# vpc-ccg/freddie

Measured on AMD Instinct MI355X. Metric: reads segmented/sec (whole node), higher is better.
Workload: dtype u32

## Files before the change

freddie_amd/csrc/freddie_seg.hip:

```cpp
#include "seg_kernels.h"

using namespace fseg;

namespace {

struct DevBuf {
    void *p = nullptr;
    size_t cap = 0;
    template <typename T> T *as() const { return reinterpret_cast<T *>(p); }
};
struct Slab {
    void *p = nullptr;
    size_t cap = 0;
};
struct HostBuf {
    void *p = nullptr;
    size_t cap = 0;
    template <typename T> T *as() const { return reinterpret_cast<T *>(p); }
};
struct Carve {
    struct Item { DevBuf *b; size_t off, bytes; };
    std::vector<Item> items;
    size_t total = 0;
    size_t add(DevBuf &b, size_t bytes) {
// ... 20 lines not shown
    SEG_POST1 = 8u,
    SEG_POST2 = 16u,
    SEG_STATUS = 32u,
    SEG_ALL = 63u,
};

}

hipError_t fseg_sort_pairs(void *tmp, size_t *tmp_bytes, const unsigned long long *keys_in, unsigned long long *keys_out,
                           const int *vals_in, int *vals_out, size_t n, unsigned end_bit, hipStream_t stream);

struct fseg_ctx {
    int device = 0;
    hipStream_t stream = nullptr;
    std::string err;
    bool have_params = false, have_batch = false, ran = false, pending = false;
    bool fetched = false;
    fseg_params P{};
    std::vector<double> w_main, w_refine, h_table;
    int n_part = 0;
    i64 K = 0, R = 0, I = 0, NPOS = 0, LANES = 0;
    i64 max_part_pos = 0;
    int thr_part = -1;
    i64 max_part_lanes = 0;
    int n_tiles = 0;
    bool expanded = false;
    std::vector<i64> part_iv_off, part_rep_off;
    Slab slab_in, slab_pos, slab_arena;
    HostBuf h_stage;
    HostBuf h_res;
    size_t res_off[4] = {0, 0, 0, 0};
    std::vector<i64> res_pfo;
    DevBuf d_labels;
    DevBuf d_packed;
    int fetched_packed = -1;
    bool label_packed_ok = true;
    bool label_has2 = false;
    bool run_label_packed = false;
    bool labels_unpacked = false;
    DevBuf d_sort_tmp;
    DevBuf d_part_iv_off, d_part_rep_off, d_part_lane_off, d_iv_start, d_iv_end, d_pos_off, d_iv_part,
        d_rep_exon_off, d_rep_weight, d_ex_ts, d_ex_te, d_tile_desc, d_iv_tile0, d_blk_iv0, d_rb_part, d_rb_r0, d_rb_sum, d_rb_base, d_rb_max, d_rb_cmax,
        d_hc_part, d_hc_p0, d_hc_n, d_hc_glo, d_hc_ghi;
    DevBuf d_lane_ex, d_lane_start, d_lane_pmax, d_hc_llo, d_hc_lhi, d_key_a, d_key_b, d_val_a, d_val_b, d_rep_last;
    DevBuf d_lane_lx, d_lex, d_rb_esum, d_rb_ebase;
    i64 max_rep_exons = 0;
    DevBuf d_w_main, d_w_refine, d_h_table, d_thr_tab;
    DevBuf d_bits;
    DevBuf d_y_raw, d_y, d_v, d_scan_state, d_bsum, d_bsum_side, d_g, d_pk, d_pf, d_kp;
    int n_hist_chunks = 0;
    DevBuf d_voff, d_chunk_off, d_csum, d_mean, d_thr, d_label_off, d_part_has2;
    int n_rep_blocks = 0;
    DevBuf d_cand_off, d_cand_y, d_fixed0, d_added, d_fixed, d_chosen, d_final_off, d_final_y, d_final_pos, d_final_iv, d_col_thr,
        d_col_zero;
    DevBuf d_tile_defer;
    DevBuf d_blk_pre, d_tile_tot, d_seg_iv, d_seg_prev, d_rseg_c, d_cand_pn, d_cand_ll, d_cand_ln, d_cand_wide, d_prob_bs;
    DevBuf d_prob_iv, d_prob_start, d_prob_n, d_prob_pair_off, d_prob_tri_off, d_prob_flags, d_prob_chain,
        d_prob_cov_off, d_prob_lane_lo, d_prob_lane_n;
    DevBuf d_dp_items, d_solve_items, d_solve_desc, d_prob_desc, d_work_pc, d_cls_items, d_work_active, d_pair_thr, d_amb, d_out, d_cov;
    DevBuf d_wide_items;
    DevBuf d_wide_all;
    DevBuf d_dpx;
    i64 dpx_base[3] = {0, 0, 0}, dpx_stride[3] = {0, 0, 0}, dpx_n[3] = {0, 0, 0};
    int dpx_nm = 0, dpx_cnt[3] = {1, 1, 1};
    static constexpr i64 kWideOneMax = 256;
    int split_dp = 7;
    i64 prob_cap = 0, work_cap = 0, pair_cap = 0, tri_cap = 0, label_cap = 0, chunk_cap = 0, cov_cap = 0;
    DevBuf d_status, d_prep, d_tacc;
    DevBuf d_sync;
    unsigned sync_gen = 0;
    unsigned sync_ticks = 1000000u;
    unsigned sync_timeouts = 0;
    unsigned forked_runs = 0;
    bool run_events_only = false;
    bool dev_sync = true;
    Status *h_status = nullptr;
    PrepStatus *h_prep = nullptr;
    bool prep_checked = false;
    bool counted_in_flight = false, counted_live = false;
    bool side_probed = false;
    bool side_ok[3] = {false, false, false};
    unsigned probe_gen = 0;
    bool owns_device = false;
    int hsa_agent = -1;
    hsa_signal_t hsa_sig = {0};
    int hsa_cpu = 0;
    const void *hsa_dst_base = nullptr;
    bool profiling = false;
    bool profile_all = true;
    bool have_huge = false;
    int nm_giant = 0;
    DevBuf d_giant;
    bool dp_wide_counts = false;
    int nm_big = kNMax;
    bool small_batch = false;
    bool tiny_on = false;
    bool use_graph = true;
    bool run_plain = false;
    bool run_linear = false;
    bool use_sized = true;
    static constexpr i64 kProbSelfMax = 4 * kProbBlock;
    bool prob_self_scan = false;
    i64 scan_single_max = 512;
    bool force_scan_stall = false;
    hipGraph_t graph[2] = {nullptr, nullptr};
    hipGraphExec_t graph_exec[2] = {nullptr, nullptr};
    bool profile_plain = false;
// ... 619 lines not shown
                           c->d_pair_thr.as<int2>(), c->pair_cap, c->P.min_read_support_outside, c->d_chosen.as<unsigned char>(), 0); \
              \
        hipLaunchKernelGGL((k_dp<kDpSmall, 256, OUTT>), dim3(grid_for(c->prob_cap, 1, 8192)), dim3(256),                       \
                           dp_lds_for(kDpSmall, (int)sizeof(OUTT)), q_mid, st, 0, kDpSmall, c->d_dp_items.as<int>(), pr,       \
                           c->d_prob_desc.as<ProbDesc>(), c->prob_cap, c->d_cand_off.as<i64>(), c->d_cand_y.as<int>(), c->d_iv_part.as<int>(), \
                           c->d_part_lane_off.as<i64>(), c->d_out.as<unsigned>(), c->tri_cap, c->d_amb.as<unsigned>(),        \
                           c->d_pair_thr.as<int2>(), c->pair_cap, c->P.min_read_support_outside,                              \
                           c->d_chosen.as<unsigned char>(), kDpWave, grid_for(c->prob_cap, 1, 8192), (uint4 *)nullptr, (i64)0 FSEG_TARG)
        hipStream_t q_small = c->small_batch ? s : fork(0);
        hipStream_t q_mid = c->small_batch ? s : fork(1);
        if (c->dp_wide_counts) {
            const bool wide_wg = dp_lds_for(c->nm_big, 4) + 8 * 1024 <= kLdsPerWg;
            if (!c->small_batch) { FSEG_LAUNCH_DP_WAVES(unsigned); }
            if (wide_wg) { FSEG_LAUNCH_DP(kNMax, 512, unsigned, c->nm_big, c->small_batch ? -1 : 1, 256); }
            else { FSEG_LAUNCH_DP(kNMax, 256, unsigned, c->nm_big, c->small_batch ? -1 : 1, 256); }
        } else {
            if (!c->small_batch) { FSEG_LAUNCH_DP_WAVES(unsigned short); }
            FSEG_LAUNCH_DP(kNMax, 512, unsigned short, c->nm_big, c->small_batch ? -1 : 1, 512);
        }
#undef FSEG_LAUNCH_DP
#undef FSEG_LAUNCH_DP_WAVES
        if (!c->small_batch) { join(0); join(1); }
        if (c->have_huge)
            hipLaunchKernelGGL(k_dp_huge, dim3(dp_grid < 256 ? dp_grid : 256), dim3(512), kHugeDpLds, s, st, c->d_dp_items.as<int>(),
                               pr, c->d_prob_desc.as<ProbDesc>(), c->prob_cap, c->d_cand_y.as<int>(), c->d_out.as<unsigned>(),
                               c->tri_cap, c->d_amb.as<unsigned>(), c->d_pair_thr.as<int2>(), c->pair_cap,
                               c->P.min_read_support_outside, c->d_chosen.as<unsigned char>());
        if (c->have_huge && c->nm_giant > 0 && c->d_giant.p)
            hipLaunchKernelGGL(k_dp_giant, dim3(kGiantWgs), dim3(512), giant_dp_lds(c->nm_giant), s, st, c->d_dp_items.as<int>(),
                               pr, c->d_prob_desc.as<ProbDesc>(), c->prob_cap, c->d_cand_y.as<int>(), c->d_out.as<unsigned>(),
                               c->tri_cap, c->d_amb.as<unsigned>(), c->d_pair_thr.as<int2>(), c->pair_cap,
                               c->P.min_read_support_outside, c->d_chosen.as<unsigned char>(), c->nm_giant,
                               c->d_giant.as<unsigned char>(), (i64)giant_scratch_bytes(c->nm_giant));
    }
    end(ST_DP); begin(ST_REFINE);
    hipLaunchKernelGGL(k_segments, dim3(grid_for(K, 1, 8192)), dim3(iv_threads), 0, s, K, c->d_pos_off.as<i64>(),
                       c->d_cand_off.as<i64>(), c->d_cand_y.as<int>(), c->d_y_raw.as<int>(), c->d_blk_pre.as<int>(), c->d_tile_tot.as<int>(), c->d_iv_tile0.as<int>(),
                       c->d_chosen.as<unsigned char>(), flag_final_bits, c->d_rseg_c.as<int>(),
                       c->d_seg_prev.as<int>(), st);
    hipLaunchKernelGGL(k_refine, dim3(2048), dim3(64), 0, s, st, c->d_seg_iv.as<int>(), c->d_rseg_c.as<int>(),
                       c->d_seg_prev.as<int>(), c->d_cand_y.as<int>(), c->d_pos_off.as<i64>(), c->d_y_raw.as<int>(),
                       c->d_w_refine.as<double>(), c->P.radius_refine, c->P.sigma, c->d_g.as<double>(), c->d_pk.as<int>(),
                       c->d_pf.as<unsigned char>(), c->d_kp.as<unsigned char>(), flag_final_bits);
    end(ST_REFINE); begin(ST_FINAL);
    scan_counts(s, bsum, flag_final_bits, &st->n_final, c->d_final_off.as<i64>() + K);
    hipLaunchKernelGGL(k_scan_emit<kEmitPositions>, dim3(scan_grid), dim3(256), 0, s, flag_final_bits,
                       NPOS, bsum, scan_state + 2 * scan_nb, &st->n_final, c->d_final_off.as<i64>() + K, &st->err, (const double *)nullptr, (double *)nullptr, K, c->d_pos_off.as<i64>(),
                       c->d_iv_start.as<int>(), c->d_blk_iv0.as<int>(), c->d_final_y.as<int>(), c->d_final_pos.as<int>(),
                       c->d_final_off.as<i64>(), 0, c->d_final_iv.as<int>());
    hipLaunchKernelGGL(k_label_cols, dim3(grid_for(NPOS / 8 + 1, 256, 2048)), dim3(256), 0, s, K, c->d_final_off.as<i64>(),
                       c->d_final_y.as<int>(), c->d_final_iv.as<int>(), c->d_iv_part.as<int>(), c->d_h_table.as<double>(), c->P.h_len,
                       c->P.threshold_rate, c->d_thr_tab.as<int2>(), c->d_col_thr.as<int2>(), c->d_col_zero.as<unsigned char>(),
                       c->d_part_has2.as<int>(), n_part, c->d_part_iv_off.as<i64>(), c->d_part_rep_off.as<i64>(),
                       c->d_label_off.as<i64>(), st, c->label_cap);
    end(ST_FINAL);
    }
    if (do_post2) {
    begin(ST_LABEL);
    if (c->label_cap > 0) {
        c->run_label_packed = lab_packed; c->labels_unpacked = false;
        if (lab_packed) {
            const i64 n16 = sized ? (label_fill_bytes + 15) / 16 : labels_n16;
            if (n16 > 0)
                hipLaunchKernelGGL(k_clear, dim3(grid_for(n16 / 4 + 1, 256, 4096)), dim3(256), 0, s, (Status *)nullptr, c->d_packed.as<unsigned>(), n16);
        } else if (!ride_fill) {
            const i64 n16 = sized ? (label_fill_bytes + 15) / 16 : labels_n16;
            if (n16 > 0)
                hipLaunchKernelGGL(k_label_zero, dim3(grid_for(n16 / 8 + 1, 256, 4096)), dim3(256), 0, s, c->d_labels.as<uint4>(), n16);
        }
        hipLaunchKernelGGL(k_label_reads, dim3(grid_for((i64)c->n_rep_blocks * kLabelSplit, 1, 65536)), dim3(256), 0, s, c->n_rep_blocks,
                           c->d_rb_part.as<int>(), c->d_rb_r0.as<int>(), c->d_label_off.as<i64>(), c->label_cap, n_part,
                           c->d_part_iv_off.as<i64>(), c->d_part_rep_off.as<i64>(), c->d_final_off.as<i64>(),
                           c->d_final_pos.as<int>(), c->d_col_thr.as<int2>(), c->d_rep_exon_off.as<i64>(),
                           c->d_ex_ts.as<int>(), c->d_ex_te.as<int>(), c->d_col_zero.as<unsigned char>(),
                           c->d_part_has2.as<int>(), c->d_labels.as<unsigned char>(), lab_packed ? c->d_packed.as<unsigned>() : (unsigned *)nullptr);
    }
    end(ST_LABEL);
    }
    if (segs & SEG_STATUS) HIP_TRY(c, hipMemcpyAsync(c->h_status, st, sizeof(Status), hipMemcpyDeviceToHost, s));
    HIP_TRY(c, fj_err);
    HIP_TRY(c, hipGetLastError());
    return FSEG_OK;
}

hipError_t wait_stream(fseg_ctx *c) {
    const auto t0 = std::chrono::steady_clock::now();
    for (;;) {
        hipError_t e = hipStreamQuery(c->stream);
        if (e != hipErrorNotReady) { (void)hipGetLastError(); return e; }
        if (std::chrono::steady_clock::now() - t0 > std::chrono::milliseconds(2)) break;
    }
    (void)hipGetLastError();
    return hipStreamSynchronize(c->stream);
}

int check_prep(fseg_ctx *c) {
    if (c->prep_checked) return FSEG_OK;
    c->prep_checked = true;
    const PrepStatus &ps = *c->h_prep;
    if (!ps.err) return FSEG_OK;
    int q = 0;
    for (int i = 1; i < 4; ++i) if (((ps.err >> i) & 1u) && (!((ps.err >> q) & 1u) || ps.bad_rep[i] < ps.bad_rep[q])) q = i;
    if (!((ps.err >> q) & 1u)) for (q = 0; q < 4 && !((ps.err >> q) & 1u); ++q) {}
    const long long r = (long long)ps.bad_rep[q];
    c->have_batch = false;
    switch (1u << q) {
        case kPrepExonEnds: return fail(c, FSEG_ERR_INPUT, "rep %lld: exon with start >= end (py/freddie_segment.py:160)", r);
        case kPrepExonOrder: return fail(c, FSEG_ERR_INPUT, "rep %lld: exons out of order (py/freddie_segment.py:158)", r);
        case kPrepExonInterval: return fail(c, FSEG_ERR_INPUT, "rep %lld: an exon does not lie inside one tint interval (py/freddie_segment.py:668)", r);
        default: return fail(c, FSEG_ERR_INPUT, "rep %lld has no exons", r);
    }
}

int run_input_errors(fseg_ctx *c, const Status &s) {
    if (s.err & kErrExonInterval) return fail(c, FSEG_ERR_INPUT, "an exon does not lie inside one tint interval (py/freddie_segment.py:668)");
    if (s.err & kErrBreakAssert) return fail(c, FSEG_ERR_INPUT, "break_large_problems: candidate window out of range or no positive signal (py/freddie_segment.py:640-643)");
    if (s.err & kErrWideMissed) return fail(c, FSEG_ERR_HIP, "internal: a problem keeps more reads than were counted for it (kErrWideMissed)");
    if (s.err & kErrProblemTooLarge) return fail(c, FSEG_ERR_UNSUPPORTED, "a DP problem has more than %d candidates (max_problem_size beyond 1000 is not supported)", kNGiant);
    return FSEG_OK;
}

int prepare_giant(fseg_ctx *c, int max_n) {
    if (max_n <= kNHuge || max_n > kNGiant) { if (max_n <= kNHuge) c->nm_giant = 0; return FSEG_OK; }
    int want = (max_n + 7) & ~7;
    if (want > kNGiant) want = kNGiant;
    if (want > c->nm_giant || c->nm_giant == 0) { c->nm_giant = want; drop_graph(c); }
    TRY(ensure(c, c->d_giant, (size_t)kGiantWgs * giant_scratch_bytes(c->nm_giant)));
    const hipError_t e = hipFuncSetAttribute(reinterpret_cast<const void *>(k_score_giant), hipFuncAttributeMaxDynamicSharedMemorySize, (int)giant_score_lds(kNGiant));
// ... 603 lines not shown
            TRY(ensure(c, c->d_sort_tmp, tmp_bytes));
            HIP_TRY(c, fseg_sort_pairs(c->d_sort_tmp.p, &tmp_bytes, c->d_key_a.as<u64>(), c->d_key_b.as<u64>(), c->d_val_a.as<int>(),
                                       c->d_val_b.as<int>(), (size_t)R, end_bit, s));
        }
        if (sort_here) {
            hipLaunchKernelGGL(k_lanes, dim3(grid_for(np, 1, 65536)), dim3(256), 0, s, np, c->d_part_rep_off.as<i64>(), c->d_part_lane_off.as<i64>(),
                               c->d_key_b.as<u64>(), c->d_val_b.as<int>(), c->d_rep_weight.as<int>(), c->d_rep_last.as<int>(),
                               c->d_rep_exon_off.as<i64>(), c->d_lane_ex.as<longlong2>(), c->d_lane_start.as<int>(), c->d_lane_pmax.as<int>(),
                               1, c->d_key_a.as<u64>(), c->d_ex_ts.as<int>(), c->d_ex_te.as<int>(), c->d_lane_lx.as<int2>(), c->d_lex.as<int2>());
        } else {
            const int rbg = grid_for(n_rep_blocks, 1, 65536);
            hipLaunchKernelGGL(k_lane_blocks, dim3(rbg), dim3(256), 0, s, (int)n_rep_blocks, c->d_rb_part.as<int>(), c->d_rb_r0.as<int>(),
                               c->d_part_rep_off.as<i64>(), c->d_val_b.as<int>(), c->d_rep_weight.as<int>(), c->d_rep_last.as<int>(),
                               c->d_rb_sum.as<i64>(), c->d_rb_max.as<int>(), c->d_rep_exon_off.as<i64>(), c->d_rb_esum.as<i64>());
            hipLaunchKernelGGL(k_lane_block_scan, dim3(grid_for(np, 4, 4096)), dim3(256), 0, s, np, (int)n_rep_blocks, c->d_rb_part.as<int>(),
                               c->d_part_lane_off.as<i64>(), c->d_rb_sum.as<i64>(), c->d_rb_max.as<int>(), c->d_rb_base.as<i64>(),
                               c->d_rb_cmax.as<int>(), c->d_part_rep_off.as<i64>(), c->d_rep_exon_off.as<i64>(), c->d_rb_esum.as<i64>(),
                               c->d_rb_ebase.as<i64>());
            hipLaunchKernelGGL(k_lane_emit, dim3(rbg), dim3(256), 0, s, (int)n_rep_blocks, c->d_rb_part.as<int>(), c->d_rb_r0.as<int>(),
                               c->d_part_rep_off.as<i64>(), c->d_key_b.as<u64>(), c->d_val_b.as<int>(), c->d_rep_weight.as<int>(),
                               c->d_rep_last.as<int>(), c->d_rep_exon_off.as<i64>(), c->d_rb_base.as<i64>(), c->d_rb_cmax.as<int>(),
                               c->d_lane_ex.as<longlong2>(), c->d_lane_start.as<int>(), c->d_lane_pmax.as<int>(), c->d_rb_ebase.as<i64>(),
                               c->d_ex_ts.as<int>(), c->d_ex_te.as<int>(), c->d_lane_lx.as<int2>(), c->d_lex.as<int2>());
        }
    }
    hipLaunchKernelGGL(k_hist_ranges, dim3(grid_for(n_chunks, 256, 4096)), dim3(256), 0, s, (int)n_chunks, c->d_hc_part.as<int>(),
                       c->d_hc_glo.as<int>(), c->d_hc_ghi.as<int>(), c->d_part_lane_off.as<i64>(), c->d_lane_start.as<int>(),
                       c->d_lane_pmax.as<int>(), c->d_hc_llo.as<i64>(), c->d_hc_lhi.as<i64>());
    HIP_TRY(c, hipMemcpyAsync(c->h_prep, c->d_prep.p, sizeof(PrepStatus), hipMemcpyDeviceToHost, s));
    HIP_TRY(c, hipGetLastError());
    {
        const size_t np8 = (size_t)NPOS + 64;
        auto atleast = [](i64 &cap, i64 v) { if (cap < v) cap = v; };
        atleast(c->chunk_cap, NPOS / 8192 + np + 8);
        Carve cv;
        cv.add(c->d_y_raw, np8 * 4); cv.add(c->d_y, np8 * 8); cv.add(c->d_bits, 3 * flag_words(np8) * 4);
        cv.add(c->d_v, np8 * 8);
        cv.add(c->d_scan_state, ((size_t)nb * 3 + 1) * 8);
        cv.add(c->d_bsum, ((size_t)nb + 2) * 4);
        cv.add(c->d_bsum_side, ((size_t)nb + 2) * 4);
        cv.add(c->d_g, np8 * 8); cv.add(c->d_pk, np8 * 4); cv.add(c->d_pf, np8); cv.add(c->d_kp, np8);
        cv.add(c->d_part_has2, ((size_t)np + 1) * 4);
        cv.add(c->d_tile_tot, ((size_t)n_tiles + 1) * 4);
        cv.add(c->d_blk_pre, ((size_t)n_tiles + 1) * (kSmoothTile / kSumBlock) * 4);
        cv.add(c->d_tile_defer, ((size_t)n_tiles + 1) * 4);
        cv.add(c->d_voff, ((size_t)np + 2) * 8); cv.add(c->d_chunk_off, ((size_t)np + 2) * 8);
        cv.add(c->d_mean, ((size_t)np + 1) * 8); cv.add(c->d_thr, ((size_t)np + 1) * 8);
        cv.add(c->d_label_off, ((size_t)np + 2) * 8);
        cv.add(c->d_csum, (size_t)c->chunk_cap * 16);
        cv.add(c->d_cand_off, ((size_t)K + 2) * 8); cv.add(c->d_final_off, ((size_t)K + 2) * 8);
        cv.add(c->d_cand_y, np8 * 4); cv.add(c->d_fixed0, np8); cv.add(c->d_added, np8);
        cv.add(c->d_fixed, np8); cv.add(c->d_chosen, np8);
        cv.add(c->d_final_y, np8 * 4); cv.add(c->d_final_pos, np8 * 4); cv.add(c->d_final_iv, np8 * 4); cv.add(c->d_col_thr, np8 * 8); cv.add(c->d_col_zero, np8);
        cv.add(c->d_seg_iv, np8 * 4); cv.add(c->d_seg_prev, np8 * 4); cv.add(c->d_rseg_c, np8 * 4);
        cv.add(c->d_cand_pn, np8 * 4); cv.add(c->d_cand_ll, np8 * 4); cv.add(c->d_cand_ln, np8 * 4); cv.add(c->d_cand_wide, np8);
        cv.add(c->d_prob_bs, ((size_t)NPOS / kProbBlock + 2) * kProbCols * 8);
        TRY(reserve(c, c->slab_pos, cv.total));
        cv.bind(c->slab_pos);
        atleast(c->prob_cap, 1024); atleast(c->work_cap, 1024); atleast(c->pair_cap, 1 << 16); atleast(c->tri_cap, 1 << 18);
        atleast(c->label_cap, 1 << 16); atleast(c->cov_cap, 1 << 18);
        TRY(alloc_arenas(c));
    }
    drop_graph(c);
    c->have_batch = true;
    if (c->trace)
        fprintf(stderr, "[fseg] upload: plan %.3f ms, tables %.3f ms, copy-in %.3f ms (%.1f MB), enqueue %.3f ms; %lld positions, %lld reps, %lld exons\n",
                t_plan, t_tables, t_copy, up_bytes / 1e6, tk.ms(), (long long)NPOS, (long long)R, (long long)I);
    return FSEG_OK;
}

static int run_impl(fseg_ctx *c);
int fseg_run(fseg_ctx *c) {
    const int rc = run_impl(c);
    if (rc != FSEG_OK && c && !c->pending) set_in_flight(c, false);
    return rc;
}
static int run_impl(fseg_ctx *c) {
    if (!c) return FSEG_ERR_ARG;
    if (!c->have_params || !c->have_batch) return fail(c, FSEG_ERR_ARG, "fseg_run: set parameters and upload a batch first");
    HIP_TRY(c, hipSetDevice(c->device));
    if (c->pending) TRY(finish_run(c));
    c->fetched = false;
    c->run_events_only = false;
    set_in_flight(c, true);
    claim_device(c);
    if (c->owns_device) ++c->forked_runs;
    if (c->use_fork && !c->side[0] && c->owns_device) {
        hipStream_t made[fseg_ctx::kSide] = {};
        hipError_t e = hipSuccess;
        for (int i = 0; e == hipSuccess && i < fseg_ctx::kSide; ++i) e = hipStreamCreateWithFlags(&made[i], hipStreamNonBlocking);
        if (e != hipSuccess) {
            for (hipStream_t m : made) if (m) (void)hipStreamDestroy(m);
            return fail(c, FSEG_ERR_HIP, "hipStreamCreateWithFlags: %s", hipGetErrorString(e));
        }
        for (int i = 0; i < fseg_ctx::kSide; ++i) c->side[i] = made[i];
    }
    if (c->owns_device && c->dev_sync && !c->side_probed) TRY(probe_side_queues(c));
    if (!c->ran && c->use_sized) return run_sized(c);
    if (c->label_cap > 0) {
        void *before[2] = {c->d_labels.p, c->d_packed.p};
        TRY(ensure_label_arena(c));
        if (before[0] != c->d_labels.p || before[1] != c->d_packed.p) drop_graph(c);
    }
    c->last_sized = false;
    c->run_plain = !c->use_graph || c->profile_plain || would_fork(c);
    if (!c->run_plain) {
// ... 333 lines not shown
```

freddie_amd/csrc/seg_common.h:

```cpp
#pragma once
#include <hip/hip_runtime.h>
#include <type_traits>
#include <hsa/hsa.h>
#include <hsa/hsa_ext_amd.h>
#include <chrono>
#include <algorithm>
#include <atomic>
#include <mutex>
#include <cmath>
#include <cstdarg>
#include <cstdio>
#include <cstdlib>
#include <cstring>
#include <string>
#include <vector>

#include "freddie_seg.h"

namespace fseg {


typedef long long i64;

typedef unsigned long long u64;
// ... 1138 lines not shown
__host__ __device__ inline size_t dpx_in_bytes(int nm) { return ((size_t)nm * (nm - 1) / 2 * 4 + 15) & ~(size_t)15; }

inline size_t dpx_slot_bytes(int nm, int cnt_bytes) {
    const size_t tri = (size_t)nm * (nm - 1) * (nm - 2) / 6;
    return (kDpxHeader + dpx_in_bytes(nm) + ((tri * cnt_bytes + 15) & ~(size_t)15) + 255) & ~(size_t)255;
}

inline size_t solve_lds_for(int nm, int cov_stride, int cnt_bytes) {
    const size_t tri = (size_t)nm * (nm - 1) * (nm - 2) / 6;
    return (solve_shared_bytes(nm, cov_stride) + ((tri + 15) & ~(size_t)15) * cnt_bytes + 15) & ~(size_t)15;
}


constexpr i64 kSplitGridCap = 1 << 20;

inline size_t dpw_lds_for(int nm, int key_bytes, int cnt_bytes) {
    const size_t pairs = (size_t)nm * (nm - 1) / 2, tri = (size_t)nm * (nm - 1) * (nm - 2) / 6;
    return ((pairs * key_bytes + 15) & ~(size_t)15) + ((pairs * 4 + 15) & ~(size_t)15) + ((pairs + 15) & ~(size_t)15) + ((tri * cnt_bytes + 15) & ~(size_t)15);
}


constexpr int kHugeSub = 32;

constexpr size_t kHugeScoreLds = (size_t)(kNHuge * (kNHuge - 1) / 2) * 8 + (size_t)kHugeSub * (kNHuge + 1) * 4;


constexpr size_t kHugeDpLds = (size_t)(kNHuge * (kNHuge - 1) / 2) * (8 + 4 + 1) + 16;


constexpr int kGiantWgs = 64;

inline size_t giant_score_lds(int nm) { return (size_t)(2 * nm + kHugeSub * (nm + 1)) * 4; }

inline size_t giant_dp_lds(int nm) { return (size_t)nm * 4; }

inline size_t giant_scratch_bytes(int nm) {
    const size_t pairs = (size_t)nm * (nm - 1) / 2;
    return ((pairs * (8 + 4 + 2) + 255) & ~(size_t)255);
}


constexpr int kSegChunks = 4;


constexpr int kRefCap = 1024;

constexpr int kLabelCols = 1024;

#ifndef FSEG_LABEL_STAGE
#define FSEG_LABEL_STAGE 1024
#endif
constexpr int kLabelStage = FSEG_LABEL_STAGE;

constexpr int kLabelSplit = 4;


enum : unsigned { kPrepExonEnds = 1u, kPrepExonOrder = 2u, kPrepExonInterval = 4u, kPrepNoExons = 8u };

struct PrepStatus {
    unsigned err;
    unsigned pad;
    i64 bad_rep[4];
};


constexpr int kLaneSortMax = 2048;

constexpr int kLexChunk = 4096;

__device__ __forceinline__ void lex_copy_tile(int eb, int ne, i64 src0, int tot_e, i64 tile_e0, const int *__restrict__ ex_ts,
                                              const int *__restrict__ ex_te, int2 *__restrict__ lex, unsigned char *owner_s ,
                                              int *eb_s , i64 *src_s ) {
    eb_s[threadIdx.x] = eb; src_s[threadIdx.x] = src0;
    for (int c0 = 0; c0 < tot_e; c0 += kLexChunk) {
        __syncthreads();
        const int lo = max(eb, c0), hi = min(eb + ne, c0 + kLexChunk);
        for (int o = lo; o < hi; ++o) owner_s[o - c0] = (unsigned char)threadIdx.x;
        __syncthreads();
        const int end = min(tot_e, c0 + kLexChunk);
        for (int o = c0 + (int)threadIdx.x; o < end; o += 256) {
            const int u = owner_s[o - c0];
            const i64 src = src_s[u] + (o - eb_s[u]);
            lex[tile_e0 + o] = make_int2(ex_ts[src], ex_te[src]);
        }
    }
    __syncthreads();
}

struct PairTable { unsigned short v[kNMax * (kNMax - 1) / 2]; };
constexpr PairTable make_pair_table() {
    PairTable t{};
    int q = 0;
    for (int j = 1; j < kNMax; ++j) for (int i = 0; i < j; ++i) t.v[q++] = (unsigned short)(i | (j << 8));
    return t;
}
static __device__ const PairTable g_pair_table = make_pair_table();
#define g_pair_ij g_pair_table.v

}
```

freddie_amd/csrc/seg_kernels.h:

```cpp
#pragma once
#include "seg_common.h"

namespace fseg {

__global__ void __launch_bounds__(256) k_thr_table(const double *h_table, int h_len, double tau, int2 *tab);

__global__ void __launch_bounds__(512) k_hist(int n_chunks, const int *chunk_part, const i64 *chunk_p0, const int *chunk_n,
                                              const int *chunk_glo, const int *chunk_ghi, const i64 *chunk_lane_lo,
                                              const i64 *chunk_lane_hi, const i64 *part_iv_off,
                                              const int *iv_start, const int *iv_end, const i64 *pos_off,
                                              const i64 *part_lane_off, const int2 *__restrict__ lane_lx, const int *lane_start,
                                              const int *lane_pmax, const int2 *__restrict__ lex,
                                              int ignore_ends, int *y_raw, Status *st, u64 *zero_ptr, i64 zero_n);

template <int R>
#ifndef FSEG_SMOOTH_OCC
#define FSEG_SMOOTH_OCC 6
#endif
__global__ void __launch_bounds__(kSmoothThreads, FSEG_SMOOTH_OCC) k_smooth(int n_tiles, const TileDesc *__restrict__ tiles,
                                                const int *__restrict__ y_raw, const double *__restrict__ w_g, int radius_rt,
                                                double *y_out, unsigned *flag_pos, unsigned *flag_cand, int *blk_pre, int *tile_tot,
                                                int *tile_defer);

__global__ void __launch_bounds__(256) k_clear(Status *st, unsigned *bits, i64 n_words);
// ... 103 lines not shown
__global__ void __launch_bounds__(64) k_wait_word(Status *st, const unsigned *words, unsigned mask, unsigned gen, unsigned max_ticks);

__global__ void __launch_bounds__(64) k_signal(unsigned *word, unsigned gen);
__global__ void __launch_bounds__(64) k_probe_wait(const unsigned *word, unsigned gen, unsigned *result, unsigned max_ticks);

template <int NM, typename CntT, typename V, bool SPLIT>
__global__ void __launch_bounds__(SolveCfg<NM>::kThreads, SolveCfg<NM>::kMinBlocks) k_solve(Status *st, int cls, int nm, i64 lb_h, i64 ln_h, ProblemArrays pr,
                                                                  const ProbDesc *desc, i64 prob_cap, const int *cand_y,
                                                                  const int2 *__restrict__ lane_lx, const int2 *__restrict__ lex,
                                                                  const double *h_table, int h_len, double tau, const int2 *thr_tab,
                                                                  int support, unsigned char *chosen,
                                                                  unsigned char *dpx, i64 dpx_stride,
                                                                  const int *__restrict__ wide_items FSEG_TPARAM);

template <int NM, typename OutT, typename V, int T>
__global__ void __launch_bounds__(T) k_dpw(Status *st, int nm, i64 list_base, i64 list_n, ProblemArrays pr, const ProbDesc *desc,
                                            const unsigned char *dpx, i64 dpx_stride,
                                            int support, unsigned char *chosen, const int *__restrict__ wide_items FSEG_TPARAM);

__global__ void __launch_bounds__(512) k_score_huge(Status *st, const int *dp_items, ProblemArrays pr, const ProbDesc *desc,
                                                    i64 prob_cap, i64 work_cap, const int *cand_y, const unsigned *cov_g,
                                                    i64 cov_cap, const int2 *pair_thr, i64 pair_cap, unsigned *out_g,
                                                    i64 tri_cap, unsigned *amb_g);

__global__ void __launch_bounds__(512) k_dp_huge(Status *st, const int *dp_items, ProblemArrays pr, const ProbDesc *desc,
                                                 i64 prob_cap, const int *cand_y, const unsigned *out_g, i64 tri_cap,
                                                 const unsigned *amb_g, const int2 *pair_thr, i64 pair_cap, int support,
                                                 unsigned char *chosen);

__global__ void __launch_bounds__(512) k_score_giant(Status *st, const int *dp_items, ProblemArrays pr, const ProbDesc *desc,
                                                     i64 prob_cap, i64 work_cap, const int *cand_y, const unsigned *cov_g,
                                                     i64 cov_cap, const int2 *pair_thr, i64 pair_cap, unsigned *out_g,
                                                     i64 tri_cap, unsigned *amb_g, int nm, unsigned char *scratch, i64 scratch_stride);

__global__ void __launch_bounds__(512) k_dp_giant(Status *st, const int *dp_items, ProblemArrays pr, const ProbDesc *desc,
                                                  i64 prob_cap, const int *cand_y, const unsigned *out_g, i64 tri_cap,
                                                  const unsigned *amb_g, const int2 *pair_thr, i64 pair_cap, int support,
                                                  unsigned char *chosen, int nm, unsigned char *scratch, i64 scratch_stride);

__global__ void k_segments(i64 K, const i64 *pos_off, const i64 *cand_off, const int *cand_y, const int *__restrict__ y_raw,
                           const int *__restrict__ blk_pre, const int *tile_tot, const int *iv_tile0, const unsigned char *chosen, unsigned *final_flag, int *rseg_c, int *rseg_prev,
                           Status *st);

__global__ void __launch_bounds__(64) k_refine(const Status *st, const int *cand_iv, const int *rseg_c,
                                               const int *rseg_prev, const int *cand_y, const i64 *pos_off,
                                               const int *y_raw, const double *w_g, int radius, double sigma,
                                               double *g_scr, int *pk_scr, unsigned char *flag_scr,
                                               unsigned char *keep_scr, unsigned *final_flag);

__global__ void __launch_bounds__(256) k_label_cols(i64 K, const i64 *final_off, const int *final_y, const int *final_iv, const int *iv_part,
                                                    const double *h_table, int h_len, double tau, const int2 *thr_tab, int2 *col_thr,
                                                    unsigned char *col_zero, int *part_has2, int n_part,
                                                    const i64 *part_iv_off, const i64 *part_rep_off, i64 *label_off,
                                                    Status *st, i64 label_cap);

__global__ void __launch_bounds__(256) k_label_zero(uint4 *labels16, i64 n16);

__global__ void __launch_bounds__(256) k_label_reads(int n_blocks, const int *rb_part, const int *rb_r0,
                                                     const i64 *label_off, i64 label_cap, int n_part,
                                                     const i64 *part_iv_off, const i64 *part_rep_off,
                                                     const i64 *final_off, const int *final_pos, const int2 *col_thr,
                                                     const i64 *rep_exon_off, const int *ex_ts, const int *ex_te,
                                                     const unsigned char *col_zero, const int *part_has2,
                                                     unsigned char *labels, unsigned *packed);
__global__ void __launch_bounds__(256) k_unpack_labels(const unsigned *__restrict__ packed, uint4 *__restrict__ labels16, i64 n16);

__global__ void __launch_bounds__(256) k_pack_labels(const uint4 *__restrict__ labels16, unsigned *__restrict__ packed, i64 n16);

__global__ void __launch_bounds__(256) k_prep_reps(int n_blocks, const int *rb_part, const int *rb_r0, const i64 *part_rep_off,
                                                   const i64 *part_iv_off, const int *iv_start, const int *iv_end,
                                                   const i64 *rep_exon_off, const int *ex_ts, const int *ex_te, u64 *key,
                                                   int *val, int *rep_last, PrepStatus *ps);

__global__ void __launch_bounds__(256) k_lanes(int n_part, const i64 *part_rep_off, const i64 *part_lane_off, const u64 *key_sorted,
                                               const int *val_sorted, const int *rep_weight, const int *rep_last,
                                               const i64 *rep_exon_off, longlong2 *lane_ex, int *lane_start, int *lane_pmax,
                                               int sort_here, const u64 *key_unsorted, const int *ex_ts, const int *ex_te,
                                               int2 *lane_lx, int2 *lex);

__global__ void __launch_bounds__(256) k_lane_blocks(int n_blocks, const int *rb_part, const int *rb_r0, const i64 *part_rep_off,
                                                     const int *val_sorted, const int *rep_weight, const int *rep_last,
                                                     i64 *rb_sum, int *rb_max, const i64 *rep_exon_off, i64 *rb_esum);

__global__ void __launch_bounds__(256) k_lane_block_scan(int n_part, int n_blocks, const int *rb_part, const i64 *part_lane_off,
                                                         const i64 *rb_sum, const int *rb_max, i64 *rb_base, int *rb_cmax,
                                                         const i64 *part_rep_off, const i64 *rep_exon_off, const i64 *rb_esum, i64 *rb_ebase);

__global__ void __launch_bounds__(256) k_lane_emit(int n_blocks, const int *rb_part, const int *rb_r0, const i64 *part_rep_off,
                                                   const u64 *key_sorted, const int *val_sorted, const int *rep_weight, const int *rep_last,
                                                   const i64 *rep_exon_off, const i64 *rb_base, const int *rb_cmax,
                                                   longlong2 *lane_ex, int *lane_start, int *lane_pmax, const i64 *rb_ebase,
                                                   const int *ex_ts, const int *ex_te, int2 *lane_lx, int2 *lex);

__global__ void __launch_bounds__(256) k_hist_ranges(int n_chunks, const int *hc_part, const int *hc_glo, const int *hc_ghi,
                                                     const i64 *part_lane_off, const int *lane_start, const int *lane_pmax,
                                                     i64 *hc_llo, i64 *hc_lhi);

}
```

freddie_amd/csrc/seg_tail.hip:

```cpp
#include "seg_kernels.h"

namespace fseg {

__global__ void k_segments(i64 K, const i64 *pos_off, const i64 *cand_off, const int *cand_y, const int *__restrict__ y_raw,
                           const int *__restrict__ blk_pre, const int *tile_tot, const int *iv_tile0, const unsigned char *chosen, unsigned *final_flag, int *rseg_c, int *rseg_prev,
                           Status *st) {
    __shared__ int lds[16];
    __shared__ int cnt_s[16];
    __shared__ u64 base_s;
    const int T = blockDim.x;
    int lane = lane_id(), wave = threadIdx.x >> 6, nw = (T + 63) >> 6;
    auto inner_sum_ok = [&](i64 base, int tile0, int py, int y) -> bool {
        const int a = py + 20, b = y - 21;
        const int ta = a >> kSmoothShift, tb = b >> kSmoothShift;
        if (tb - ta > 64) return true;
        constexpr int kBlocks = kSmoothTile / kSumBlock;
        const int *tt = tile_tot + tile0;
        const int *yr = y_raw + base;
        const int a0 = a & ~(kSumBlock - 1), b0 = b & ~(kSumBlock - 1);
        i64 tot = (i64)blk_pre[(i64)(tile0 + tb) * kBlocks + ((b & (kSmoothTile - 1)) >> kSumShift)]
                - (i64)blk_pre[(i64)(tile0 + ta) * kBlocks + ((a & (kSmoothTile - 1)) >> kSumShift)];
        int4u va[kSumBlock / 4], vb[kSumBlock / 4];
#pragma unroll
        for (int e = 0; e < kSumBlock / 4; ++e) { va[e] = *reinterpret_cast<const int4u *>(yr + a0 + 4 * e); vb[e] = *reinterpret_cast<const int4u *>(yr + b0 + 4 * e); }
// ... 230 lines not shown
            if (bq < 0) break;
            if (lane == 0) {
                kp[bq] = 2;
                int pj = pk[bq];
                for (int q = bq - 1; q >= 0 && pj - pk[q] < skip; --q) kp[q] = 0;
                for (int q = bq + 1; q < m && pk[q] - pj < skip; ++q) kp[q] = 0;
            }
            __syncthreads();
        }
        for (int q = lane; q < m; q += 64) {
            if (kp[q] != 2) continue;
            int i = pk[q];
            i64 a = (i64)rint((double)i - sigma), b = (i64)rint((double)i + sigma + 1.0);
            if (a < 0) { a += len; if (a < 0) a = 0; } else if (a > len) a = len;
            if (b < 0) { b += len; if (b < 0) b = 0; } else if (b > len) b = len;
            double sm = 0.0;
            for (i64 x = a; x < b; ++x) sm = __dadd_rn(sm, g[x]);
            if (!(sm < 20.0)) set_flag(final_flag, base + i);
        }
        __syncthreads();
      }
    }
}


__device__ void label_plan(int n_part, const i64 *part_iv_off, const i64 *part_rep_off,
                           const i64 *final_off, i64 *label_off, Status *st, i64 label_cap) {
    __shared__ i64 carry_s;
    __shared__ i64 scan_lds[16];
    if (threadIdx.x == 0) carry_s = 0;
    __syncthreads();
    for (int p0 = 0; p0 < n_part; p0 += blockDim.x) {
        int p = p0 + threadIdx.x;
        i64 bytes = 0;
        if (p < n_part) {
            i64 F = final_off[part_iv_off[p + 1]] - final_off[part_iv_off[p]];
            bytes = (part_rep_off[p + 1] - part_rep_off[p]) * (F > 0 ? F - 1 : 0);
        }
        i64 tot;
        const i64 ex = wg_exclusive_scan64(bytes, scan_lds, &tot);
        const i64 carry = carry_s;
        if (p < n_part) label_off[p] = carry + ex;
        __syncthreads();
        if (threadIdx.x == 0) carry_s = carry + tot;
        __syncthreads();
    }
    if (threadIdx.x == 0) {
        label_off[n_part] = carry_s;
        st->label_bytes = (u64)carry_s;
        if (carry_s > label_cap) atomicOr(&st->err, kErrOverflowLabels);
    }
}

__global__ void __launch_bounds__(256) k_label_cols(i64 K, const i64 *final_off, const int *final_y, const int *final_iv, const int *iv_part,
                                                    const double *h_table, int h_len, double tau, const int2 *thr_tab, int2 *col_thr,
                                                    unsigned char *col_zero, int *part_has2, int n_part,
                                                    const i64 *part_iv_off, const i64 *part_rep_off, i64 *label_off,
                                                    Status *st, i64 label_cap) {
    if (blockIdx.x == 0) label_plan(n_part, part_iv_off, part_rep_off, final_off, label_off, st, label_cap);
    i64 F = final_off[K];
    for (i64 f = (i64)blockIdx.x * blockDim.x + threadIdx.x; f < F; f += (i64)gridDim.x * blockDim.x) {
        const i64 k = final_iv[f];
        if (f + 1 == final_off[k + 1]) { col_thr[f] = make_int2(0x7fffffff, 0x7fffffff); col_zero[f] = '0'; continue; }
        int hi, lo;
        label_thresholds_tab((i64)final_y[f + 1] - final_y[f] + 1, thr_tab, h_table, h_len, tau, &hi, &lo);
        col_thr[f] = make_int2(hi, lo);
        col_zero[f] = lo >= 0 ? '0' : '2';
        if (lo < 0) atomicOr(&part_has2[iv_part[k]], 1);
    }
}

__global__ void __launch_bounds__(256) k_label_zero(uint4 *labels16, i64 n16) {
    fill_labels(labels16, n16, (i64)blockIdx.x * blockDim.x + threadIdx.x, (i64)gridDim.x * blockDim.x);
}

__global__ void __launch_bounds__(256) k_label_reads(int n_blocks, const int *rb_part, const int *rb_r0,
                                                     const i64 *label_off, i64 label_cap, int n_part,
                                                     const i64 *part_iv_off, const i64 *part_rep_off,
                                                     const i64 *final_off, const int *final_pos, const int2 *col_thr,
                                                     const i64 *rep_exon_off, const int *ex_ts, const int *ex_te,
                                                     const unsigned char *col_zero, const int *part_has2,
                                                     unsigned char *labels, unsigned *packed) {
    __shared__ int fp_s[kLabelCols + 1];
    __shared__ int2 th_s[kLabelCols];
    if (label_off[n_part] > label_cap) return;
    for (i64 unit = blockIdx.x; unit < (i64)n_blocks * kLabelSplit; unit += gridDim.x) {
        const int blk = (int)(unit / kLabelSplit), sub = (int)(unit % kLabelSplit);
        int p = rb_part[blk];
        i64 f0 = final_off[part_iv_off[p]];
        i64 F = final_off[part_iv_off[p + 1]] - f0;
        i64 S = F - 1;
        if (S <= 0) continue;
        if ((i64)rb_r0[blk] + sub * (256 / kLabelSplit) >= part_rep_off[p + 1]) continue;
        const int *fp = final_pos + f0;
        const int2 *th = col_thr + f0;
        __syncthreads();
        if (S <= kLabelStage) {
            for (int x = threadIdx.x; x <= S; x += blockDim.x) fp_s[x] = fp[x];
            for (int x = threadIdx.x; x < S; x += blockDim.x) th_s[x] = th[x];
            fp = fp_s; th = th_s;
        }
        __syncthreads();
        i64 r = (i64)rb_r0[blk] + sub * (256 / kLabelSplit) + (threadIdx.x / kLabelSplit);
        const int q = threadIdx.x % kLabelSplit;
#ifdef FSEG_LAB_NOSEARCH
        if (fp[0] != -12345) continue;
#endif
        if (!packed && part_has2[p]) {
            if (r < part_rep_off[p + 1]) {
                unsigned char *row0 = labels + label_off[p] + (r - part_rep_off[p]) * S;
                const unsigned char *cz = col_zero + f0;
                for (i64 x = S * q / kLabelSplit; x < S * (q + 1) / kLabelSplit; ++x) row0[x] = cz[x];
            }
            __threadfence_block();
            __syncthreads();
        }
        if (r >= part_rep_off[p + 1]) continue;
        const i64 row_g0 = label_off[p] + (r - part_rep_off[p]) * S;
        unsigned char *row = labels + row_g0;
        unsigned acc = 0;
        i64 acc_w = -1;
        i64 e = rep_exon_off[r], e1 = rep_exon_off[r + 1];
        if (e >= e1) continue;
        int first_ts = ex_ts[e], last_te = ex_te[e1 - 1];
        int lo = 0, hi = (int)S;
        while (lo < hi) { int mid = (lo + hi) >> 1; if (fp[mid + 1] <= first_ts) lo = mid + 1; else hi = mid; }
        int c_hi = lo; hi = (int)S;
        while (c_hi < hi) { int mid = (c_hi + hi) >> 1; if (fp[mid] <= last_te) c_hi = mid + 1; else hi = mid; }
        const int span = c_hi - lo;
        const int c_a = lo + (int)((i64)span * q / kLabelSplit), c_b = lo + (int)((i64)span * (q + 1) / kLabelSplit);
        if (c_a >= c_b) continue;
#ifdef FSEG_LAB_NOLOOP
        if (c_a != -12345) { if (c_b == 0x7ffffff0) atomicOr(&packed[0], 1u); continue; }
#endif
        if (q) {
            const int g = fp[c_a];
            i64 a = e, b = e1;
            while (a < b) { i64 mid = (a + b) >> 1; if (ex_te[mid] < g) a = mid + 1; else b = mid; }
            e = a;
        }
        int ts = 0, te = 0;
        if (e < e1) { ts = ex_ts[e]; te = ex_te[e]; }
        for (int c = c_a; c < c_b; ++c) {
            int2 t2 = th[c];
            if (t2.x == 0x7fffffff) continue;
            int g0 = fp[c], g1 = fp[c + 1];
            while (e < e1 && te < g0) { ++e; if (e < e1) { ts = ex_ts[e]; te = ex_te[e]; } }
            int cov = 0;
            if (e < e1 && ts < g1) {
                int a = ts > g0 ? ts : g0, b2 = te + 1 < g1 ? te + 1 : g1;
                if (b2 > a) cov += b2 - a;
                for (i64 x = e + 1; x < e1 && ex_ts[x] < g1; ++x) {
                    int a3 = ex_ts[x] > g0 ? ex_ts[x] : g0;
                    int b3 = ex_te[x] + 1 < g1 ? ex_te[x] + 1 : g1;
                    if (b3 > a3) cov += b3 - a3;
                }
            }
            const unsigned char lab = cov >= t2.x ? '1' : (cov <= t2.y ? '0' : '2');
            if (lab != (t2.y < 0 ? '2' : '0')) {
                if (packed) {
                    const i64 g = row_g0 + c, w = g >> 4;
#ifdef FSEG_LAB_NOSTORE
                    if (w != acc_w) { acc_w = w; }
#else
                    if (w != acc_w) { if (acc) atomicOr(&packed[acc_w], acc); acc_w = w; acc = 0; }
#endif
                    acc |= (unsigned)(lab - '0') << (2 * (int)(g & 15));
                } else row[c] = lab;
            }
        }
        if (acc) atomicOr(&packed[acc_w], acc);
    }
}




__global__ void __launch_bounds__(256) k_unpack_labels(const unsigned *__restrict__ packed, uint4 *__restrict__ labels16, i64 n16) {
    for (i64 i = (i64)blockIdx.x * blockDim.x + threadIdx.x; i < n16; i += (i64)gridDim.x * blockDim.x) {
        const unsigned v = packed[i];
        unsigned w[4];
#pragma unroll
        for (int q = 0; q < 4; ++q) {
            const unsigned b = (v >> (8 * q)) & 0xffu;
            w[q] = 0x30303030u | (b & 3u) | ((b & 0xcu) << 6) | ((b & 0x30u) << 12) | ((b & 0xc0u) << 18);
        }
        labels16[i] = make_uint4(w[0], w[1], w[2], w[3]);
    }
}
__global__ void __launch_bounds__(256) k_pack_labels(const uint4 *__restrict__ labels16, unsigned *__restrict__ packed, i64 n16) {
    for (i64 i = (i64)blockIdx.x * blockDim.x + threadIdx.x; i < n16; i += (i64)gridDim.x * blockDim.x) {
        const uint4 v = labels16[i];
        const unsigned w[4] = {v.x, v.y, v.z, v.w};
        unsigned out = 0;
#pragma unroll
        for (int q = 0; q < 4; ++q) {
            const unsigned x = w[q] & 0x03030303u;
            out |= ((x & 3u) | ((x >> 6) & 0xcu) | ((x >> 12) & 0x30u) | ((x >> 18) & 0xc0u)) << (8 * q);
        }
        packed[i] = out;
    }
}

}
```

Measured before the change: 577.0 million.

## Precompute full-coverage column label masks and span-fill interior exon columns in packed labeling

k_label_cols now also computes, per column, the label code a read would get if it fully covered that column, and packs these codes 16 per word into a new col_full bitmap using wave shuffles. In the packed path, k_label_reads walks exons instead of columns. It computes exact coverage only for each exon's boundary columns and copies the interior columns' labels from the precomputed masks with shifted word operations. k_label_reads is templated on packed versus unpacked. The goal is to cut the per-column coverage loop for long exons, at the cost of a binary search per exon, an extra buffer and more code.

Result: no change. 571.8 million (-0.9%).

```diff
diff --git a/freddie_amd/csrc/freddie_seg.hip b/freddie_amd/csrc/freddie_seg.hip
--- a/freddie_amd/csrc/freddie_seg.hip
+++ b/freddie_amd/csrc/freddie_seg.hip
@@ -96,7 +96,7 @@
     DevBuf d_voff, d_chunk_off, d_csum, d_mean, d_thr, d_label_off, d_part_has2;
     int n_rep_blocks = 0;
     DevBuf d_cand_off, d_cand_y, d_fixed0, d_added, d_fixed, d_chosen, d_final_off, d_final_y, d_final_pos, d_final_iv, d_col_thr,
-        d_col_zero;
+        d_col_zero, d_col_full;
     DevBuf d_tile_defer;
     DevBuf d_blk_pre, d_tile_tot, d_seg_iv, d_seg_prev, d_rseg_c, d_cand_pn, d_cand_ll, d_cand_ln, d_cand_wide, d_prob_bs;
     DevBuf d_prob_iv, d_prob_start, d_prob_n, d_prob_pair_off, d_prob_tri_off, d_prob_flags, d_prob_chain,
@@ -822,7 +822,7 @@
                        c->d_final_y.as<int>(), c->d_final_iv.as<int>(), c->d_iv_part.as<int>(), c->d_h_table.as<double>(), c->P.h_len,
                        c->P.threshold_rate, c->d_thr_tab.as<int2>(), c->d_col_thr.as<int2>(), c->d_col_zero.as<unsigned char>(),
                        c->d_part_has2.as<int>(), n_part, c->d_part_iv_off.as<i64>(), c->d_part_rep_off.as<i64>(),
-                       c->d_label_off.as<i64>(), st, c->label_cap);
+                       c->d_label_off.as<i64>(), st, c->label_cap, c->d_final_pos.as<int>(), c->d_col_full.as<unsigned>());
     end(ST_FINAL);
     }
     if (do_post2) {
@@ -838,12 +838,14 @@
             if (n16 > 0)
                 hipLaunchKernelGGL(k_label_zero, dim3(grid_for(n16 / 8 + 1, 256, 4096)), dim3(256), 0, s, c->d_labels.as<uint4>(), n16);
         }
-        hipLaunchKernelGGL(k_label_reads, dim3(grid_for((i64)c->n_rep_blocks * kLabelSplit, 1, 65536)), dim3(256), 0, s, c->n_rep_blocks,
+        auto label_reads = lab_packed ? k_label_reads<true> : k_label_reads<false>;
+        hipLaunchKernelGGL(label_reads, dim3(grid_for((i64)c->n_rep_blocks * kLabelSplit, 1, 65536)), dim3(256), 0, s, c->n_rep_blocks,
                            c->d_rb_part.as<int>(), c->d_rb_r0.as<int>(), c->d_label_off.as<i64>(), c->label_cap, n_part,
                            c->d_part_iv_off.as<i64>(), c->d_part_rep_off.as<i64>(), c->d_final_off.as<i64>(),
                            c->d_final_pos.as<int>(), c->d_col_thr.as<int2>(), c->d_rep_exon_off.as<i64>(),
                            c->d_ex_ts.as<int>(), c->d_ex_te.as<int>(), c->d_col_zero.as<unsigned char>(),
-                           c->d_part_has2.as<int>(), c->d_labels.as<unsigned char>(), lab_packed ? c->d_packed.as<unsigned>() : (unsigned *)nullptr);
+                           c->d_part_has2.as<int>(), c->d_labels.as<unsigned char>(), lab_packed ? c->d_packed.as<unsigned>() : (unsigned *)nullptr,
+                           c->d_col_full.as<unsigned>());
     }
     end(ST_LABEL);
     }
@@ -1553,6 +1555,7 @@
         cv.add(c->d_cand_y, np8 * 4); cv.add(c->d_fixed0, np8); cv.add(c->d_added, np8);
         cv.add(c->d_fixed, np8); cv.add(c->d_chosen, np8);
         cv.add(c->d_final_y, np8 * 4); cv.add(c->d_final_pos, np8 * 4); cv.add(c->d_final_iv, np8 * 4); cv.add(c->d_col_thr, np8 * 8); cv.add(c->d_col_zero, np8);
+        cv.add(c->d_col_full, label_full_words(np8) * 4);
         cv.add(c->d_seg_iv, np8 * 4); cv.add(c->d_seg_prev, np8 * 4); cv.add(c->d_rseg_c, np8 * 4);
         cv.add(c->d_cand_pn, np8 * 4); cv.add(c->d_cand_ll, np8 * 4); cv.add(c->d_cand_ln, np8 * 4); cv.add(c->d_cand_wide, np8);
         cv.add(c->d_prob_bs, ((size_t)NPOS / kProbBlock + 2) * kProbCols * 8);
diff --git a/freddie_amd/csrc/seg_common.h b/freddie_amd/csrc/seg_common.h
--- a/freddie_amd/csrc/seg_common.h
+++ b/freddie_amd/csrc/seg_common.h
@@ -1214,7 +1214,13 @@
 #endif
 constexpr int kLabelStage = FSEG_LABEL_STAGE;
 
-constexpr int kLabelSplit = 4;
+#ifndef FSEG_LABEL_SPLIT
+#define FSEG_LABEL_SPLIT 4
+#endif
+constexpr int kLabelSplit = FSEG_LABEL_SPLIT;
+
+constexpr int kLabelFullPad = 1;
+inline size_t label_full_words(size_t n_final_cap) { return n_final_cap / 16 + 8; }
 
 
 enum : unsigned { kPrepExonEnds = 1u, kPrepExonOrder = 2u, kPrepExonInterval = 4u, kPrepNoExons = 8u };
diff --git a/freddie_amd/csrc/seg_kernels.h b/freddie_amd/csrc/seg_kernels.h
--- a/freddie_amd/csrc/seg_kernels.h
+++ b/freddie_amd/csrc/seg_kernels.h
@@ -179,17 +179,18 @@
                                                     const double *h_table, int h_len, double tau, const int2 *thr_tab, int2 *col_thr,
                                                     unsigned char *col_zero, int *part_has2, int n_part,
                                                     const i64 *part_iv_off, const i64 *part_rep_off, i64 *label_off,
-                                                    Status *st, i64 label_cap);
+                                                    Status *st, i64 label_cap, const int *final_pos, unsigned *col_full);
 
 __global__ void __launch_bounds__(256) k_label_zero(uint4 *labels16, i64 n16);
 
+template <bool kPacked>
 __global__ void __launch_bounds__(256) k_label_reads(int n_blocks, const int *rb_part, const int *rb_r0,
                                                      const i64 *label_off, i64 label_cap, int n_part,
                                                      const i64 *part_iv_off, const i64 *part_rep_off,
                                                      const i64 *final_off, const int *final_pos, const int2 *col_thr,
                                                      const i64 *rep_exon_off, const int *ex_ts, const int *ex_te,
                                                      const unsigned char *col_zero, const int *part_has2,
-                                                     unsigned char *labels, unsigned *packed);
+                                                     unsigned char *labels, unsigned *packed, const unsigned *col_full);
 __global__ void __launch_bounds__(256) k_unpack_labels(const unsigned *__restrict__ packed, uint4 *__restrict__ labels16, i64 n16);
 
 __global__ void __launch_bounds__(256) k_pack_labels(const uint4 *__restrict__ labels16, unsigned *__restrict__ packed, i64 n16);
diff --git a/freddie_amd/csrc/seg_tail.hip b/freddie_amd/csrc/seg_tail.hip
--- a/freddie_amd/csrc/seg_tail.hip
+++ b/freddie_amd/csrc/seg_tail.hip
@@ -306,21 +306,36 @@
     }
 }
 
+__device__ __forceinline__ unsigned label_code(int cov, int2 t2) {
+    const unsigned char lab = cov >= t2.x ? '1' : (cov <= t2.y ? '0' : '2');
+    return lab != (t2.y < 0 ? '2' : '0') ? (unsigned)(lab - '0') : 0u;
+}
+
 __global__ void __launch_bounds__(256) k_label_cols(i64 K, const i64 *final_off, const int *final_y, const int *final_iv, const int *iv_part,
                                                     const double *h_table, int h_len, double tau, const int2 *thr_tab, int2 *col_thr,
                                                     unsigned char *col_zero, int *part_has2, int n_part,
                                                     const i64 *part_iv_off, const i64 *part_rep_off, i64 *label_off,
-                                                    Status *st, i64 label_cap) {
+                                                    Status *st, i64 label_cap, const int *final_pos, unsigned *col_full) {
     if (blockIdx.x == 0) label_plan(n_part, part_iv_off, part_rep_off, final_off, label_off, st, label_cap);
     i64 F = final_off[K];
-    for (i64 f = (i64)blockIdx.x * blockDim.x + threadIdx.x; f < F; f += (i64)gridDim.x * blockDim.x) {
-        const i64 k = final_iv[f];
-        if (f + 1 == final_off[k + 1]) { col_thr[f] = make_int2(0x7fffffff, 0x7fffffff); col_zero[f] = '0'; continue; }
-        int hi, lo;
-        label_thresholds_tab((i64)final_y[f + 1] - final_y[f] + 1, thr_tab, h_table, h_len, tau, &hi, &lo);
-        col_thr[f] = make_int2(hi, lo);
-        col_zero[f] = lo >= 0 ? '0' : '2';
-        if (lo < 0) atomicOr(&part_has2[iv_part[k]], 1);
+    for (i64 f = (i64)blockIdx.x * blockDim.x + threadIdx.x; f - (threadIdx.x & 15) < F; f += (i64)gridDim.x * blockDim.x) {
+        unsigned code = 0;
+        if (f < F) {
+            const i64 k = final_iv[f];
+            if (f + 1 == final_off[k + 1]) { col_thr[f] = make_int2(0x7fffffff, 0x7fffffff); col_zero[f] = '0'; }
+            else {
+                int hi, lo;
+                label_thresholds_tab((i64)final_y[f + 1] - final_y[f] + 1, thr_tab, h_table, h_len, tau, &hi, &lo);
+                col_thr[f] = make_int2(hi, lo);
+                col_zero[f] = lo >= 0 ? '0' : '2';
+                if (lo < 0) atomicOr(&part_has2[iv_part[k]], 1);
+                const int cov = final_pos[f + 1] - final_pos[f];
+                code = label_code(cov, make_int2(hi, lo));
+            }
+        }
+        unsigned v = code << (2 * (int)(f & 15));
+        v |= __shfl_xor(v, 1); v |= __shfl_xor(v, 2); v |= __shfl_xor(v, 4); v |= __shfl_xor(v, 8);
+        if ((f & 15) == 0) col_full[kLabelFullPad + (f >> 4)] = v;
     }
 }
 
@@ -328,15 +343,17 @@
     fill_labels(labels16, n16, (i64)blockIdx.x * blockDim.x + threadIdx.x, (i64)gridDim.x * blockDim.x);
 }
 
+template <bool kPacked>
 __global__ void __launch_bounds__(256) k_label_reads(int n_blocks, const int *rb_part, const int *rb_r0,
                                                      const i64 *label_off, i64 label_cap, int n_part,
                                                      const i64 *part_iv_off, const i64 *part_rep_off,
                                                      const i64 *final_off, const int *final_pos, const int2 *col_thr,
                                                      const i64 *rep_exon_off, const int *ex_ts, const int *ex_te,
                                                      const unsigned char *col_zero, const int *part_has2,
-                                                     unsigned char *labels, unsigned *packed) {
+                                                     unsigned char *labels, unsigned *packed, const unsigned *col_full) {
     __shared__ int fp_s[kLabelCols + 1];
     __shared__ int2 th_s[kLabelCols];
+    __shared__ unsigned tm_s[kPacked ? kLabelCols / 16 + 4 : 1];
     if (label_off[n_part] > label_cap) return;
     for (i64 unit = blockIdx.x; unit < (i64)n_blocks * kLabelSplit; unit += gridDim.x) {
         const int blk = (int)(unit / kLabelSplit), sub = (int)(unit % kLabelSplit);
@@ -348,11 +365,18 @@
         if ((i64)rb_r0[blk] + sub * (256 / kLabelSplit) >= part_rep_off[p + 1]) continue;
         const int *fp = final_pos + f0;
         const int2 *th = col_thr + f0;
+        const unsigned *tm = col_full;
+        i64 tm0 = 0;
         __syncthreads();
         if (S <= kLabelStage) {
             for (int x = threadIdx.x; x <= S; x += blockDim.x) fp_s[x] = fp[x];
             for (int x = threadIdx.x; x < S; x += blockDim.x) th_s[x] = th[x];
             fp = fp_s; th = th_s;
+            if (kPacked) {
+                tm0 = f0 >> 4;
+                for (int x = threadIdx.x; x < (int)(S >> 4) + 4; x += blockDim.x) tm_s[x] = col_full[tm0 + x];
+                tm = tm_s;
+            }
         }
         __syncthreads();
         i64 r = (i64)rb_r0[blk] + sub * (256 / kLabelSplit) + (threadIdx.x / kLabelSplit);
@@ -360,7 +384,7 @@
 #ifdef FSEG_LAB_NOSEARCH
         if (fp[0] != -12345) continue;
 #endif
-        if (!packed && part_has2[p]) {
+        if (!kPacked && part_has2[p]) {
             if (r < part_rep_off[p + 1]) {
                 unsigned char *row0 = labels + label_off[p] + (r - part_rep_off[p]) * S;
                 const unsigned char *cz = col_zero + f0;
@@ -371,9 +395,6 @@
         }
         if (r >= part_rep_off[p + 1]) continue;
         const i64 row_g0 = label_off[p] + (r - part_rep_off[p]) * S;
-        unsigned char *row = labels + row_g0;
-        unsigned acc = 0;
-        i64 acc_w = -1;
         i64 e = rep_exon_off[r], e1 = rep_exon_off[r + 1];
         if (e >= e1) continue;
         int first_ts = ex_ts[e], last_te = ex_te[e1 - 1];
@@ -385,7 +406,7 @@
         const int c_a = lo + (int)((i64)span * q / kLabelSplit), c_b = lo + (int)((i64)span * (q + 1) / kLabelSplit);
         if (c_a >= c_b) continue;
 #ifdef FSEG_LAB_NOLOOP
-        if (c_a != -12345) { if (c_b == 0x7ffffff0) atomicOr(&packed[0], 1u); continue; }
+        if (c_a != -12345) { if (c_b == 0x7ffffff0) labels[0] = 1; continue; }
 #endif
         if (q) {
             const int g = fp[c_a];
@@ -395,9 +416,7 @@
         }
         int ts = 0, te = 0;
         if (e < e1) { ts = ex_ts[e]; te = ex_te[e]; }
-        for (int c = c_a; c < c_b; ++c) {
-            int2 t2 = th[c];
-            if (t2.x == 0x7fffffff) continue;
+        auto column_cov = [&](int c) -> int {
             int g0 = fp[c], g1 = fp[c + 1];
             while (e < e1 && te < g0) { ++e; if (e < e1) { ts = ex_ts[e]; te = ex_te[e]; } }
             int cov = 0;
@@ -410,22 +429,78 @@
                     if (b3 > a3) cov += b3 - a3;
                 }
             }
-            const unsigned char lab = cov >= t2.x ? '1' : (cov <= t2.y ? '0' : '2');
-            if (lab != (t2.y < 0 ? '2' : '0')) {
-                if (packed) {
-                    const i64 g = row_g0 + c, w = g >> 4;
+            return cov;
+        };
+        auto label_exact = [&](int c) -> unsigned {
+            const int2 t2 = th[c];
+            if (t2.x == 0x7fffffff) return 0u;
+            return label_code(column_cov(c), t2);
+        };
+        if (kPacked) {
+            unsigned acc = 0;
+            i64 acc_w = -1;
 #ifdef FSEG_LAB_NOSTORE
-                    if (w != acc_w) { acc_w = w; }
+            unsigned sink = 0;
+            auto put = [&](i64 w, unsigned bits) { if (w != acc_w) { sink ^= acc; acc_w = w; acc = 0; } acc |= bits; };
 #else
-                    if (w != acc_w) { if (acc) atomicOr(&packed[acc_w], acc); acc_w = w; acc = 0; }
-#endif
-                    acc |= (unsigned)(lab - '0') << (2 * (int)(g & 15));
-                } else row[c] = lab;
-            }
-        }
-        if (acc) atomicOr(&packed[acc_w], acc);
-    }
-}
+            auto put = [&](i64 w, unsigned bits) { if (w != acc_w) { if (acc) atomicOr(&packed[acc_w], acc); acc_w = w; acc = 0; } acc |= bits; };
+#endif
+            const i64 d = row_g0 - f0;
+            const int sh2 = 2 * (int)((0 - d) & 15);
+            int c = c_a;
+            for (i64 x = e; x < e1 && c < c_b; ++x) {
+                const int xs = ex_ts[x], xt = ex_te[x];
+                if (xs >= fp[c_b]) break;
+                if (xt < fp[c]) continue;
+                int a = c, b = c_b - 1;
+                while (a < b) { int mid = (a + b) >> 1; if (fp[mid + 1] <= xs) a = mid + 1; else b = mid; }
+                const int cs = a;
+                b = c_b - 1;
+                while (a < b) { int mid = (a + b + 1) >> 1; if (fp[mid] <= xt) a = mid; else b = mid - 1; }
+                const int ce = a;
+#ifndef FSEG_LAB_NOEXACT
+                { const unsigned k = label_exact(cs); if (k) { const i64 g = row_g0 + cs; put(g >> 4, k << (2 * (int)(g & 15))); } }
+#endif
+#ifndef FSEG_LAB_NOSPAN
+                if (ce > cs + 1) {
+                    const i64 ga = row_g0 + cs + 1, gb = row_g0 + ce;
+                    for (i64 w = ga >> 4; w <= (gb - 1) >> 4; ++w) {
+                        const int lb = ga > (w << 4) ? (int)(ga - (w << 4)) : 0, hb = gb - (w << 4) < 16 ? (int)(gb - (w << 4)) : 16;
+                        const unsigned m = (hb == 16 ? ~0u : (1u << (2 * hb)) - 1u) & ~((1u << (2 * lb)) - 1u);
+                        const i64 j = kLabelFullPad + (((w << 4) - d) >> 4) - tm0;
+                        const u64 t = (u64)tm[j] | ((u64)tm[j + 1] << 32);
+                        const unsigned bits = (unsigned)(t >> sh2) & m;
+                        if (bits) put(w, bits);
+                    }
+                }
+#endif
+#ifndef FSEG_LAB_NOEXACT
+                if (ce > cs) { const unsigned k = label_exact(ce); if (k) { const i64 g = row_g0 + ce; put(g >> 4, k << (2 * (int)(g & 15))); } }
+#endif
+                c = ce + 1;
+            }
+#ifdef FSEG_LAB_NOSTORE
+            if ((sink ^ acc) == 0x9e3779b9u) atomicOr(&packed[acc_w], acc);
+#else
+            if (acc) atomicOr(&packed[acc_w], acc);
+#endif
+        } else {
+            unsigned char *row = labels + row_g0;
+            for (int c = c_a; c < c_b; ++c) {
+                int2 t2 = th[c];
+                if (t2.x == 0x7fffffff) continue;
+                const int cov = column_cov(c);
+                const unsigned char lab = cov >= t2.x ? '1' : (cov <= t2.y ? '0' : '2');
+                if (lab != (t2.y < 0 ? '2' : '0')) row[c] = lab;
+            }
+        }
+    }
+}
+
+__attribute__((used)) static const void *const kLabelInstances[] = {
+    reinterpret_cast<const void *>(&k_label_reads<true>),
+    reinterpret_cast<const void *>(&k_label_reads<false>),
+};
 
 
 
```
